# anonymous-author-918/deq-mpc-corl

Hardware: AMD Instinct MI355X
Metric: QP solves/sec at (B,T=20,nx=13,nu=4) (higher is better)
Workload: dtype f32

## Files before the change

### deq-mpc-corl_amd/csrc/alqp_kernels.hip

```cpp
#include <hip/hip_runtime.h>

#include "alqp_team.hpp"
#include "alqp_quad.hpp"
#include "mi_alqp.h"
#include "alqp_dims.hpp"

#ifndef ALQP_PART
#define ALQP_PART 0
#endif
#define ALQP_BUILD_MAIN (ALQP_PART == 0 || ALQP_PART == 1)
#define ALQP_BUILD_QUAD (ALQP_PART == 0 || ALQP_PART == 2 || ALQP_PART == 3)
#define ALQP_QUAD_F32 (ALQP_PART == 0 || ALQP_PART == 2)
#define ALQP_QUAD_F64 (ALQP_PART == 0 || ALQP_PART == 3)

#include <hip/hip_cooperative_groups.h>

namespace alqp {

template <typename real>
struct SolveArgs {
    int B, T;
    int al_iter, max_newton, n_ls, flags;
    real rho_scale;
    const real *Qd, *q, *F, *c, *x0, *ulo, *uhi;
// ... 335 lines not shown
#endif
    QSTAMP(-1);
    if (!(a.flags & ALQP_WS_PRIMED)) {
        if constexpr (NL) qd.stage_in(false, false);
        else qd.stage_in(a.max_newton == 0 || a.al_iter == 0 || (a.flags & ALQP_EXIT_IN_KERNEL) ||
                         (!C::PHI0_FWD && (a.flags & ALQP_INIT_MERIT)));
    }
    const bool ref_exit = (a.flags & ALQP_EXIT_IN_KERNEL) != 0;
    int gphase = 0;

    int step_id = 0;
    bool pend = false;
    real alpha_pend = 0;
    int bad = 0;
    real rn2 = 0, phi_next = 0;
    for (int it = 0; it < a.al_iter; ++it) {
        bool phi_from_forward = false;
        if (a.flags & ALQP_INIT_MERIT) {
            if (it > 0) {
                phi_prev = phi_next;
            } else if (C::PHI0_FWD && a.max_newton > 0 && !ref_exit) {
                phi_from_forward = true;
            } else {
                if constexpr (NL) qd.template linearize<Dyn>(real(0), false);
                real p1[1];
                qd.template merit_candidates<1>(p1, true);
                phi_prev = p1[0];
            }
        }
        pend = false;
        double nrm_old = 0;
        int n_done = 0;
        if (ref_exit) {
            int bad0 = 0;
            const real r0 = it == 0 ? qd.rplus2(bad0) : rn2;
            nrm_old = sqrt(grid_sum_ordered(wave_sum_leaders(exit_term(r0, qor(qd.info)), active && qd.q == 0), a.exit_scratch, gphase));
        }
        for (int st = 0; st < a.max_newton; ++st, ++step_id) {
            real *tg = nullptr;
            if constexpr (TRACE) tg = (tr.g && active) ? tr.g + ((size_t)step_id * a.B + b) * T * N : nullptr;
            QSTAMP(9);
            if constexpr (NL) {
                qd.template linearize<Dyn>(alpha_pend, pend);
                pend = false;
            }
            qd.forward(tg, alpha_pend, pend, (phi_from_forward && st == 0) ? &phi_prev : nullptr);
            real ph[20];
            qd.template backward<FUSE_LS>(ph);
            QSTAMP(-1);
            if constexpr (TRACE) {
                if (tr.d && active) {
                    real *td = tr.d + ((size_t)step_id * a.B + b) * T * N;
                    for (int t = 0; t < T; ++t)
                        for (int j = qd.q; j < N; j += 4) td[t * N + j] = qd.recp(t)[C::oY + C::pn(j)];
                }
            }
            if constexpr (NL) qd.template merit_nonlin<Dyn>(ph);
            else if constexpr (!FUSE_LS) qd.template merit_candidates<20>(ph, false);
            QSTAMP(6);
            int kbest = 0;
            real best = ph[0];
#pragma unroll
            for (int k = 1; k < 20; ++k) {
                if (k < a.n_ls && !(best != best) && (ph[k] != ph[k] || ph[k] < best)) {
                    best = ph[k];
                    kbest = k;
                }
            }
            const bool acc = best < phi_prev;
            if constexpr (TRACE) {
                if (active && qd.q == 0) {
                    if (tr.phi)
#pragma unroll
                        for (int k = 0; k < 20; ++k)
                            if (k < a.n_ls) tr.phi[((size_t)step_id * a.n_ls + k) * a.B + b] = ph[k];
                    if (tr.phi_prev) tr.phi_prev[(size_t)step_id * a.B + b] = phi_prev;
                    if (tr.k) tr.k[(size_t)step_id * a.B + b] = kbest;
                    if (tr.accept) tr.accept[(size_t)step_id * a.B + b] = acc ? 1 : 0;
                }
            }
            const real alpha = acc ? real(1) / real(1 << kbest) : real(0);
            pend = true;
            alpha_pend = alpha;
            QSTAMP(7);
            phi_prev = best;
            if (ref_exit) {
                int bad1 = 0;
                real ph_unused = 0, r1 = 0;
                qd.template iter_end<Dyn>(alpha_pend, pend, false, (real)a.rho_scale, false, ph_unused, r1, bad1);
                pend = false;
                const double nw = sqrt(grid_sum_ordered(wave_sum_leaders(exit_term(r1, qor(qd.info)), active && qd.q == 0), a.exit_scratch, gphase));
                ++n_done;
                if (nw < a.exit_tol || fabs(nrm_old - nw) / nw < a.exit_tol) break;
                nrm_old = nw;
            }
        }
        if (ref_exit && a.newton_counts && blockIdx.x == 0 && lane == 0) a.newton_counts[it] = grid_barrier_timed_out(a.exit_scratch) ? -1 : n_done;
        bad = 0;
        qd.template iter_end<Dyn>(alpha_pend, pend, (a.flags & ALQP_DUAL_UPDATE) != 0, (real)a.rho_scale, it + 1 == a.al_iter,
                    phi_next, rn2, bad);
        pend = false;
    }
    if (a.al_iter <= 0) {
        rn2 = qd.rplus2(bad);
        qd.stage_out();
    }
#ifdef ALQP_PHASE_TIMING
    QSTAMP(9);
    if (lane == 0)
        for (int i = 0; i < 10; ++i) atomicAdd(&g_phase_cycles[i], qd.tacc[i]);
#endif
    if (active && qd.q == 0) {
        a.rho[b] = qd.rho;
        a.phi[b] = phi_prev;
        if (a.rnorm2) a.rnorm2[b] = rn2;
        if (a.info && qd.info && a.info[b] == 0) a.info[b] = qd.info;
        if (a.status) a.status[b] = bad ? 0 : 1;
    }
}

template <typename real, int NX, int NU>
__global__ __launch_bounds__(64) __attribute__((amdgpu_waves_per_eu(1, 1))) void k_backward_quad(BwdArgs<real> a, real *ws) {
    using C = QCfg<real, NX, NU>;
    constexpr int N = C::N;
    const int lane = threadIdx.x, qi = lane >> 2;
    const int b_raw = blockIdx.x * 16 + qi;
    const bool active = b_raw < a.B;
    const int b = active ? b_raw : a.B - 1;
    const int T = a.T;
    Quad<real, NX, NU> qd;
    __shared__ real w_lds[QCfg<real, NX, NU>::WLDS_WORDS];
    qd.wl = w_lds + threadIdx.x;
    qd.q = lane & 3;
    qd.T = T;
    qd.active = active;
    qd.gF = a.F + (size_t)b * (T - 1) * NX * N;
    qd.gQd = nullptr; qd.gq = nullptr; qd.gc = nullptr; qd.gx0 = nullptr; qd.gulo = nullptr; qd.guhi = nullptr;
    qd.st_u = 0;
    qd.gz = nullptr; qd.glam = nullptr;
    qd.rec = ws + C::rec_base(b, T);
    qd.rho = a.rho[b];
    qd.info = 0;
    qd.solve_forward(a.gbar + (size_t)b * T * N);
    real unused[20];
    qd.template backward<false>(unused);
    if (active) {
        const real *zf = a.z_final + (size_t)b * T * N;
        real *qg = a.q_grad + (size_t)b * T * N;
        real *Qg = a.Qd_grad + (size_t)b * T * N;
        for (int t = 0; t < T; ++t)
            for (int j = qd.q; j < N; j += 4) {
                const real w = qd.recp(t)[C::oY + C::pn(j)];
                qg[t * N + j] = w;
                Qg[t * N + j] = w * zf[t * N + j];
            }
    }
}

template <typename real, int NX, int NU>
__global__ __launch_bounds__(64) __attribute__((amdgpu_waves_per_eu(1, 1))) void k_newton_step_quad(StepArgs<real> a, real *ws) {
    using C = QCfg<real, NX, NU>;
    constexpr int N = C::N, SW = C::SW;
    const int lane = threadIdx.x, qi = lane >> 2;
    const int b_raw = blockIdx.x * 16 + qi;
    const bool active = b_raw < a.B;
    const int b = active ? b_raw : a.B - 1;
    const int T = a.T, M = C::M(T) + T * a.nobs;
    Quad<real, NX, NU> qd;
    __shared__ real w_lds[QCfg<real, NX, NU>::WLDS_WORDS];
    qd.wl = w_lds + threadIdx.x;
    qd.q = lane & 3;
    qd.T = T;
    qd.active = active;
    qd.gQd = a.Qd + (size_t)b * T * N;
    qd.gq = a.q + (size_t)b * T * N;
    qd.gF = a.F + (size_t)b * (T - 1) * NX * N;
    qd.gc = nullptr;
    qd.gx0 = a.x0 + (size_t)b * NX;
    qd.gulo = a.ulo + (size_t)b * a.sb_u;
    qd.guhi = a.uhi + (size_t)b * a.sb_u;
    qd.st_u = a.st_u;
    qd.gz = const_cast<real *>(a.z) + (size_t)b * T * N;
    qd.glam = const_cast<real *>(a.lam) + (size_t)b * M;
    qd.rec = ws + C::rec_base(b, T);
    qd.gFw = const_cast<real *>(qd.gF);
    qd.dyn_h = 0;
    qd.rho = a.rho[b];
    qd.info = 0;
    qd.nobs = a.nobs;
    qd.gobs = a.nobs > 0 ? a.obs + (size_t)b * T * a.nobs * 3 : nullptr;
    qd.obs_r2 = a.obs_r2;
    qd.no_init = a.no_init != 0;
    const real *gxn = a.xnext + (size_t)b * (T - 1) * NX;
    real *tg = (a.g_out && active) ? a.g_out + (size_t)b * T * N : nullptr;
    qd.template forward<true>(tg, real(0), false, nullptr, gxn);
    real unused[20];
    qd.template backward<false>(unused, a.d_out + (size_t)b * T * N);
    if (active) {
        if (qd.q == 0 && a.info && qd.info && a.info[b] == 0) a.info[b] = qd.info;
    }
}

#endif

#if ALQP_BUILD_MAIN
// ... 1217 lines not shown
```

### deq-mpc-corl_amd/csrc/alqp_quad.hpp

```cpp
#pragma once
#include <hip/hip_runtime.h>

#include "alqp_team.hpp"
#include "alqp_dyn.hpp"

namespace alqp {

template <int Q>
__device__ inline float qb(float v) {
    return __builtin_bit_cast(float, __builtin_amdgcn_mov_dpp(__builtin_bit_cast(int, v), Q * 0x55, 0xF, 0xF, true));
}
template <int Q>
__device__ inline double qb(double v) {
    long long b = __builtin_bit_cast(long long, v);
    int lo = __builtin_amdgcn_mov_dpp((int)(b & 0xffffffffll), Q * 0x55, 0xF, 0xF, true);
    int hi = __builtin_amdgcn_mov_dpp((int)(b >> 32), Q * 0x55, 0xF, 0xF, true);
    return __builtin_bit_cast(double, ((long long)hi << 32) | (unsigned int)lo);
}
template <typename real>
__device__ inline real qbv(real v, int src) {
    switch (src & 3) {
        case 0: return qb<0>(v);
        case 1: return qb<1>(v);
        case 2: return qb<2>(v);
        default: return qb<3>(v);
    }
}
template <int CTRL>
__device__ inline float qperm(float v) {
    return __builtin_bit_cast(float, __builtin_amdgcn_mov_dpp(__builtin_bit_cast(int, v), CTRL, 0xF, 0xF, true));
}
template <int CTRL>
__device__ inline double qperm(double v) {
    long long b = __builtin_bit_cast(long long, v);
    int lo = __builtin_amdgcn_mov_dpp((int)(b & 0xffffffffll), CTRL, 0xF, 0xF, true);
    int hi = __builtin_amdgcn_mov_dpp((int)(b >> 32), CTRL, 0xF, 0xF, true);
    return __builtin_bit_cast(double, ((long long)hi << 32) | (unsigned int)lo);
}
template <typename real>
__device__ inline real qsum(real v) {
    v += qperm<0xB1>(v);
    v += qperm<0x4E>(v);
    return v;
}
__device__ inline int qor(int v) {
    v |= __builtin_amdgcn_mov_dpp(v, 0xB1, 0xF, 0xF, true);
    v |= __builtin_amdgcn_mov_dpp(v, 0x4E, 0xF, 0xF, true);
    return v;
}
template <typename real>
__device__ inline real sel4(real a0, real a1, real a2, real a3, int q) {
    real lo = (q & 1) ? a1 : a0, hi = (q & 1) ? a3 : a2;
    return (q & 2) ? hi : lo;
}
// ... 14 lines not shown
}
__device__ inline void gst4(double *p, double a, double b, double c, double d) {
    d4u t; t.x = a; t.y = b; t.z = c; t.w = d;
    *reinterpret_cast<d4u *>(p) = t;
}
template <int LEN, typename real>
__device__ inline void gload(const real *p, real (&dst)[LEN]) {
#pragma unroll
    for (int c = 0; c + 4 <= LEN; c += 4) gld4(p + c, dst[c], dst[c + 1], dst[c + 2], dst[c + 3]);
#pragma unroll
    for (int c = (LEN / 4) * 4; c < LEN; ++c) dst[c] = p[c];
}

#ifndef ALQP_W_LDS
#define ALQP_W_LDS 1
#endif
#ifndef ALQP_EXP_NOQ
#define ALQP_EXP_NOQ 0
#endif
#ifndef ALQP_EXP_NORS
#define ALQP_EXP_NORS 0
#endif
#ifndef ALQP_EXP_NOL
#define ALQP_EXP_NOL 0
#endif
template <typename real, int SW, int N, bool IN_LDS>
struct WPanel {
    real a[SW][N];
    __device__ __forceinline__ real (&operator[](int s))[N] { return a[s]; }
    __device__ __forceinline__ const real (&operator[](int s) const)[N] { return a[s]; }
};
template <typename real, int N>
struct WRowLds {
    real *p;
    __device__ __forceinline__ real &operator[](int k) const { return p[k * 64]; }
};
template <typename real, int SW, int N>
struct WPanel<real, SW, N, true> {
    real *base;
    __device__ __forceinline__ WRowLds<real, N> operator[](int s) const { return WRowLds<real, N>{base + s * N * 64}; }
};
template <int LEN, typename real>
__device__ __forceinline__ void gload(const real *p, WRowLds<real, LEN> row) {
    real tmp[LEN];
    gload<LEN>(p, tmp);
#pragma unroll
    for (int k = 0; k < LEN; ++k) row[k] = tmp[k];
}

struct NoDyn {
    static constexpr int ID = 0;
};

template <typename real, int NX_, int NU_>
struct QCfg {
    static constexpr int NX = NX_, NU = NU_, N = NX_ + NU_;
    static constexpr int SH = (N + 3) / 4;
    static constexpr int SW = (NX + 3) / 4;
    static constexpr int SY = SH;
    static constexpr int HT = 2 * SH * (SH + 1);
    __host__ __device__ static constexpr int hidx(int s, int j) { return 2 * s * (s + 1) + j; }
    static constexpr int ST = 2 * SW * (SW + 1);
    static constexpr int NLAST = N - 4 * (SH - 1);
    __host__ __device__ static constexpr int lanes_of(int s) { return s == SH - 1 ? NLAST : 4; }
    __host__ __device__ static constexpr int lbase(int s) {
        int o = 0;
        for (int i = 0; i < s; ++i) o += (i + 1) * 4 * lanes_of(i);
        return o;
    }
    static constexpr int LW = lbase(SH);
    static constexpr bool PHI0_FWD = sizeof(real) == 4;
#ifndef ALQP_S_AFTER_F32
#define ALQP_S_AFTER_F32 0
#endif
    static constexpr bool S_AFTER = sizeof(real) == 8 || ALQP_S_AFTER_F32;
#ifndef ALQP_W_LDS_F32
#define ALQP_W_LDS_F32 0
#endif
    static constexpr bool W_LDS = ALQP_W_LDS && (sizeof(real) == 8 || ALQP_W_LDS_F32);
    static constexpr int WLDS_WORDS = W_LDS ? SW * N * 64 : 1;
    __host__ __device__ static constexpr int p4(int x) { return (x + 3) & ~3; }
    static constexpr int oL = 0;
    static constexpr int oY = oL + p4(LW);
    static constexpr int oR = oY + 4 * SY;
    static constexpr int oS = oR + 4 * SW;
    static constexpr int oZ = oS + 4 * SW;
    static constexpr int oLE = oZ + 4 * SY;
    static_assert(NU <= 4, "the u-slot layout holds one control per lane");
    static constexpr int oUS = oLE + 4 * SW;
    static constexpr int oQ = oUS + 16;
    static constexpr int oq = oQ + 4 * SY;
    static constexpr int oC = oq + 4 * SY;
    static constexpr int RECW = (oC + 4 * SW + 31) & ~31;
    __host__ __device__ static constexpr int pn(int k) { return (k & 3) * SY + (k >> 2); }
    __host__ __device__ static constexpr int px(int r) { return (r & 3) * SW + (r >> 2); }
    __host__ __device__ static constexpr int M(int T) { return T * NX + 2 * T * NU; }
    __host__ __device__ static constexpr size_t rec_base(int b, int T) { return (size_t)b * T * RECW; }
    __host__ __device__ static constexpr size_t ws_words(int B, int T) { return (size_t)B * T * RECW; }
    __host__ static bool ws_covers(int B, int T) { return rec_base(B - 1, T) + (size_t)(T - 1) * RECW + RECW <= ws_words(B, T); }
};

template <typename real, int NX, int NU>
struct Quad {
    using C = QCfg<real, NX, NU>;
    static constexpr int N = C::N, SH = C::SH, SW = C::SW, SY = C::SY, HT = C::HT, ST = C::ST, RECW = C::RECW;

    int q, T;
    bool active;
    const real *gQd, *gq, *gF, *gc, *gx0, *gulo, *guhi;
    long st_u;
    real *gz, *glam, *rec;
    real rho;
    int info;
    real *wl;
    using WT = WPanel<real, SW, N, C::W_LDS>;
    __device__ __forceinline__ WT wpanel() const {
        if constexpr (C::W_LDS) return WT{wl};
        else return WT{};
    }
    real *gFw;
    real dyn_h;
    const real *gobs;
    int nobs;
    real obs_r2;
    bool no_init;

    __device__ __forceinline__ real uhi(int t, int j) const { return guhi[t * st_u + j]; }
    __device__ __forceinline__ real ulo(int t, int j) const { return gulo[t * st_u + j]; }
    __device__ __forceinline__ real *recp(int t) const { return rec + (size_t)t * RECW; }
#ifdef ALQP_PHASE_TIMING
    unsigned long long tacc[10], tlast;
    __device__ __forceinline__ void stamp(int bucket) {
        unsigned long long now;
        __builtin_amdgcn_sched_barrier(0);
        asm volatile("s_waitcnt vmcnt(0)\n\ts_memtime %0\n\ts_waitcnt lgkmcnt(0)" : "=s"(now)::"memory");
        __builtin_amdgcn_sched_barrier(0);
        if (bucket >= 0) tacc[bucket] += now - tlast;
        tlast = now;
    }
#define ALQP_STAMP(b) stamp(b)
#else
#define ALQP_STAMP(b)
#endif

    __device__ __forceinline__ void ld_own_n(const real *field, real (&v)[SY]) const { gload<SY>(field + q * SY, v); }
    __device__ __forceinline__ void ld_own_x(const real *field, real (&v)[SW]) const { gload<SW>(field + q * SW, v); }
    __device__ __forceinline__ void ld_ownx_of_n(const real *field, real (&v)[SW]) const { gload<SW>(field + q * SY, v); }
    template <int LEN>
    __device__ __forceinline__ void gstore(real *p, const real (&v)[LEN]) const {
#pragma unroll
        for (int c = 0; c + 4 <= LEN; c += 4) gst4(p + c, v[c], v[c + 1], v[c + 2], v[c + 3]);
#pragma unroll
        for (int c = (LEN / 4) * 4; c < LEN; ++c) p[c] = v[c];
    }
    __device__ __forceinline__ void st_own_n(real *field, const real (&v)[SY]) const { gstore<SY>(field + q * SY, v); }
    __device__ __forceinline__ void st_own_x(real *field, const real (&v)[SW]) const { gstore<SW>(field + q * SW, v); }
    __device__ __forceinline__ void ld_rep_n(const real *field, real (&v)[N]) const {
        real w[4 * SY];
        gload<4 * SY>(field, w);
#pragma unroll
        for (int k = 0; k < N; ++k) v[k] = w[C::pn(k)];
    }
    __device__ __forceinline__ void ld_repx_of_n(const real *field, real (&v)[NX]) const {
        real w[4 * SY];
        gload<4 * SY>(field, w);
#pragma unroll
        for (int k = 0; k < NX; ++k) v[k] = w[C::pn(k)];
    }
    __device__ __forceinline__ void ld_rep_x(const real *field, real (&v)[NX]) const {
        real w[4 * SW];
        gload<4 * SW>(field, w);
#pragma unroll
        for (int r = 0; r < NX; ++r) v[r] = w[C::px(r)];
    }
    template <int LEN, int SL>
    __device__ __forceinline__ void own_of(const real (&full)[LEN], real (&v)[SL]) const {
#pragma unroll
        for (int m = 0; m < SL; ++m)
            v[m] = (4 * m < LEN) ? sel4(full[(4 * m < LEN) ? 4 * m : 0], (4 * m + 1 < LEN) ? full[(4 * m + 1 < LEN) ? 4 * m + 1 : 0] : real(0),
                                        (4 * m + 2 < LEN) ? full[(4 * m + 2 < LEN) ? 4 * m + 2 : 0] : real(0),
                                        (4 * m + 3 < LEN) ? full[(4 * m + 3 < LEN) ? 4 * m + 3 : 0] : real(0), q)
                                 : real(0);
    }
    template <int LEN, int SL>
    __device__ __forceinline__ void ld_own_ext(const real *src, real (&v)[SL]) const {
#pragma unroll
        for (int m = 0; m < SL; ++m) {
            const int k = 4 * m + q;
            const real x = src[(4 * m + 3 < LEN || k < LEN) ? k : LEN - 1];
            v[m] = (4 * m + 3 < LEN || k < LEN) ? x : real(0);
        }
    }
    template <int LEN, int SL>
    __device__ __forceinline__ void st_own_ext(real *dst, const real (&v)[SL]) const {
#pragma unroll
        for (int m = 0; m < SL; ++m)
            if (4 * m + 3 < LEN || 4 * m + q < LEN) dst[4 * m + q] = v[m];
    }

    __device__ __forceinline__ int own_ju() const { return (q - NX) & 3; }
    __device__ __forceinline__ void ld_own_us(const real *rp, real &lu, real &ll, real &bu, real &bl) const {
        gld4(rp + C::oUS + 4 * q, lu, ll, bu, bl);
    }
    __device__ __forceinline__ void ld_rep_us(const real *rp, real (&lu)[NU], real (&ll)[NU], real (&bu)[NU], real (&bl)[NU]) const {
        real w[16];
        gload<16>(rp + C::oUS, w);
#pragma unroll
        for (int ju = 0; ju < NU; ++ju) {
            const int ql = (NX + ju) & 3;
            lu[ju] = w[4 * ql];
            ll[ju] = w[4 * ql + 1];
            bu[ju] = w[4 * ql + 2];
            bl[ju] = w[4 * ql + 3];
        }
    }

    __device__ __forceinline__ void load_F_rows(int t, WT &W) const {
        const real *Fg = gF + (size_t)t * NX * N;
#pragma unroll
        for (int s = 0; s < SW; ++s) {
            const int r = 4 * s + q;
            const int rc = (4 * s + 3 < NX) ? r : (r < NX ? r : NX - 1);
            gload<N>(Fg + rc * N, W[s]);
            if (4 * s + 3 >= NX) {
                const real m = r < NX ? real(1) : real(0);
#pragma unroll
                for (int k = 0; k < N; ++k) W[s][k] *= m;
            }
        }
    }
    template <int LEN>
    __device__ __forceinline__ void copy_slice(const real *src, real *dst) const {
#pragma unroll
        for (int c = 0; 16 * c < LEN; ++c) {
            const int w0 = 16 * c + 4 * q;
            if (16 * c + 15 < LEN || w0 + 3 < LEN) {
                real a, b, cc, d;
                gld4(src + w0, a, b, cc, d);
                gst4(dst + w0, a, b, cc, d);
            } else {
#pragma unroll
                for (int w = 0; w < 4; ++w)
                    if (w0 + w < LEN) dst[w0 + w] = src[w0 + w];
            }
        }
    }
    __device__ __forceinline__ void stage_in(bool with_residual, bool have_c = true) {
#pragma unroll 2
        for (int t = 0; t < T; ++t) {
            const bool dyn = t < T - 1;
            real *rp = recp(t);
            if (active) {
                real vn[SY], vx[SW];
                ld_own_ext<N>(gz + t * N, vn);
                st_own_n(rp + C::oZ, vn);
                ld_own_ext<N>(gQd + t * N, vn);
                st_own_n(rp + C::oQ, vn);
                ld_own_ext<N>(gq + t * N, vn);
                st_own_n(rp + C::oq, vn);
                ld_own_ext<NX>(glam + t * NX, vx);
                st_own_x(rp + C::oLE, vx);
                {
                    const int ju = own_ju(), jc = ju < NU ? ju : 0;
                    const real *lb = glam + T * NX + t * 2 * NU;
                    const real a0 = lb[jc], a1 = lb[NU + jc], a2 = guhi[t * st_u + jc], a3 = gulo[t * st_u + jc];
                    const bool has = ju < NU;
                    gst4(rp + C::oUS + 4 * q, has ? a0 : real(0), has ? a1 : real(0), has ? a2 : real(0), has ? a3 : real(0));
                }
                if (dyn && have_c) ld_own_ext<NX>(gc + t * NX, vx);
                else {
#pragma unroll
                    for (int s = 0; s < SW; ++s) vx[s] = 0;
                }
                if (have_c) st_own_x(rp + C::oC, vx);
            }
            if (with_residual) {
                WT W = wpanel();
                real zt[N];
                load_F_rows(dyn ? t : (T > 1 ? T - 2 : 0), W);
                gload<N>(gz + t * N, zt);
                real rr[SW];
#pragma unroll
                for (int s = 0; s < SW; ++s) {
                    const int r = 4 * s + q;
                    rr[s] = 0;
                    if (4 * s + 3 < NX || r < NX) {
                        real xn = dyn ? gc[t * NX + r] : real(0);
#pragma unroll
                        for (int k = 0; k < N; ++k) xn = fma_(W[s][k], zt[k], xn);
                        rr[s] = dyn ? gz[(t + 1) * N + r] - xn : gz[r] - gx0[r];
                    }
                }
                if (active) st_own_x(rp + C::oR, rr);
            }
        }
    }
    __device__ __forceinline__ void stage_out() {
        if (!active) return;
#pragma unroll 2
        for (int t = 0; t < T; ++t) {
            const real *rp = recp(t);
            real vn[SY], vx[SW];
            ld_own_n(rp + C::oZ, vn);
            st_own_ext<N>(gz + t * N, vn);
            ld_own_x(rp + C::oLE, vx);
            st_own_ext<NX>(glam + t * NX, vx);
            {
                real lu, ll, bu, bl;
                ld_own_us(rp, lu, ll, bu, bl);
                const int ju = own_ju();
                if (ju < NU) {
                    glam[T * NX + t * 2 * NU + ju] = lu;
                    glam[T * NX + t * 2 * NU + NU + ju] = ll;
                }
            }
        }
    }

    template <class Dyn>
    __device__ __forceinline__ void linearize(real alpha, bool pend) {
// ... 381 lines not shown
                        real wv[KB][SW];
#pragma unroll
                        for (int kk = 0; kk < KB; ++kk)
#pragma unroll
                            for (int s = 0; s < SW; ++s)
                                if (k0 + kk < N) wv[kk][s] = W[s][k0 + kk];
                        __builtin_amdgcn_sched_barrier(0);
#pragma unroll
                        for (int kk = 0; kk < KB; ++kk) {
                            const int k = k0 + kk;
                            if (k < N) {
                                const real lkj = qbv(H[C::hidx(k >> 2, j)], k) * ip;
#pragma unroll
                                for (int s = (k >> 2); s < SH; ++s) H[C::hidx(s, k)] = fma_(-H[C::hidx(s, j)], lkj, H[C::hidx(s, k)]);
#pragma unroll
                                for (int s = 0; s < SW; ++s) W[s][k] = fma_(-wj[s], lkj, wv[kk][s]);
                                Y[k] = fma_(-Y[j], lkj, Y[k]);
                            }
                        }
                    }
                } else {
#pragma unroll
                for (int k = j + 1; k < N; ++k) {
                    const real lkj = qbv(H[C::hidx(k >> 2, j)], k) * ip;
#pragma unroll
                    for (int s = (k >> 2); s < SH; ++s) H[C::hidx(s, k)] = fma_(-H[C::hidx(s, j)], lkj, H[C::hidx(s, k)]);
#pragma unroll
                    for (int s = 0; s < SW; ++s) W[s][k] = fma_(-W[s][j], lkj, W[s][k]);
                    Y[k] = fma_(-Y[j], lkj, Y[k]);
                }
                }
                if constexpr (C::S_AFTER) ipv[j] = ip;
                if (!C::S_AFTER && dyn) {
#pragma unroll
                    for (int b = 0; b < NX; ++b) {
                        const real wbj = qbv(W[b >> 2][j], b) * ip;
#pragma unroll
                        for (int s = (b >> 2); s < SW; ++s) S[C::hidx(s, b)] = fma_(W[s][j], wbj, S[C::hidx(s, b)]);
                    }
                    const real yip = Y[j] * ip;
#pragma unroll
                    for (int s = 0; s < SW; ++s) Sy[s] = fma_(W[s][j], yip, Sy[s]);
                }
                H[C::hidx(j >> 2, j)] = (q == (j & 3)) ? ip : H[C::hidx(j >> 2, j)];
            }
            ALQP_STAMP(2);
            if (active) {
                if (!(ALQP_EXP_NOL && t >= T - ALQP_EXP_NOL))
#pragma unroll
                for (int s = 0; s < SH; ++s)
#pragma unroll
                    for (int c = 0; c <= s; ++c)
                        if (C::lanes_of(s) == 4 || q < C::lanes_of(s))
                            gst4(rp + C::oL + C::lbase(s) + c * 4 * C::lanes_of(s) + 4 * q, H[C::hidx(s, 4 * c)],
                                 H[C::hidx(s, 4 * c + 1)], H[C::hidx(s, 4 * c + 2)], H[C::hidx(s, 4 * c + 3)]);
                real yo[SY];
                own_of<N, SY>(Y, yo);
                st_own_n(rp + C::oY, yo);
                if (pending) st_own_n(rp + C::oZ, zs);
            }

            if constexpr (C::S_AFTER) {
                if (dyn) {
#pragma unroll
                    for (int j = 0; j < N; ++j) {
#pragma unroll
                        for (int b = 0; b < NX; ++b) {
                            const real wbj = qbv(W[b >> 2][j], b) * ipv[j];
#pragma unroll
                            for (int s = (b >> 2); s < SW; ++s) S[C::hidx(s, b)] = fma_(W[s][j], wbj, S[C::hidx(s, b)]);
                        }
                        const real yip = Y[j] * ipv[j];
#pragma unroll
                        for (int s = 0; s < SW; ++s) Sy[s] = fma_(W[s][j], yip, Sy[s]);
                    }
                }
            }
#pragma unroll
            for (int s = 0; s < SW; ++s) {
                vpo[s] = v[s];
                Syo[s] = Sy[s];
            }
            ALQP_STAMP(3);
        }
        if constexpr (C::PHI0_FWD) { if (phi0) *phi0 = qsum(mdist); }
    }

    template <bool LS>
    __device__ __forceinline__ void backward(real (&phi)[20], real *d_ext = nullptr) {
        constexpr int MU0 = NX / 4;
        real c0 = 0, c1 = 0, c2 = 0;
        real acc[20];
        real rvT[SW], lvT[SW];
#pragma unroll
        for (int k = 0; k < 20; ++k) acc[k] = 0;
#pragma unroll
        for (int s = 0; s < SW; ++s) rvT[s] = lvT[s] = 0;
        real dxn[NX];
#pragma unroll
        for (int j = 0; j < NX; ++j) dxn[j] = 0;
        for (int t = T - 1; t >= 0; --t) {
            const bool dyn = t < T - 1;
            real *rp = recp(t);
            real H[HT];
            if (ALQP_EXP_NOL && t >= T - ALQP_EXP_NOL) {
#pragma unroll
                for (int i = 0; i < HT; ++i) H[i] = real(1);
            } else
#pragma unroll
            for (int s = 0; s < SH; ++s)
#pragma unroll
                for (int c = 0; c <= s; ++c) {
                    const int ql = (C::lanes_of(s) == 4 || q < C::lanes_of(s)) ? q : 0;
                    gld4(rp + C::oL + C::lbase(s) + c * 4 * C::lanes_of(s) + 4 * ql, H[C::hidx(s, 4 * c)],
                         H[C::hidx(s, 4 * c + 1)], H[C::hidx(s, 4 * c + 2)], H[C::hidx(s, 4 * c + 3)]);
                }
            real yo[SY];
            ld_own_n(rp + C::oY, yo);
            real Y[N];
#pragma unroll
            for (int j = 0; j < N; ++j) Y[j] = qbv(yo[j >> 2], j);
            WT W = wpanel();
            load_F_rows(dyn ? t : (T > 1 ? T - 2 : 0), W);
            real zz[SY], QQ[SY], qq[SY], rv[SW], lv[SW];
            real lu = 0, ll = 0, bu = 0, bl = 0;
            if constexpr (LS) {
                ld_own_n(rp + C::oZ, zz);
                if constexpr (ALQP_EXP_NOQ) { for (int m = 0; m < SY; ++m) QQ[m] = real(1); }
                else ld_own_n(rp + C::oQ, QQ);
                ld_own_n(rp + C::oq, qq);
                ld_own_us(rp, lu, ll, bu, bl);
                if constexpr (ALQP_EXP_NORS) { for (int s = 0; s < SW; ++s) rv[s] = real(0); }
                else ld_own_x(rp + C::oR, rv);
                ld_own_x(rp + C::oLE, lv);
            }
            ALQP_STAMP(4);
            real dxs[SW];
#pragma unroll
            for (int s = 0; s < SW; ++s)
                dxs[s] = sel4(dxn[4 * s], (4 * s + 1 < NX) ? dxn[(4 * s + 1 < NX) ? 4 * s + 1 : 0] : real(0),
                              (4 * s + 2 < NX) ? dxn[(4 * s + 2 < NX) ? 4 * s + 2 : 0] : real(0),
                              (4 * s + 3 < NX) ? dxn[(4 * s + 3 < NX) ? 4 * s + 3 : 0] : real(0), q);
            if (dyn) {
                real vv[N];
#pragma unroll
                for (int j = 0; j < N; ++j) {
                    real p = 0;
#pragma unroll
                    for (int s = 0; s < SW; ++s) p = fma_(W[s][j], dxs[s], p);
                    vv[j] = qsum(p);
                }
#pragma unroll
                for (int j = 0; j < N; ++j) {
                    const real wj = vv[j] * qbv(H[C::hidx(j >> 2, j)], j);
#pragma unroll
                    for (int k = j + 1; k < N; ++k) vv[k] = fma_(-qbv(H[C::hidx(k >> 2, j)], k), wj, vv[k]);
                }
#pragma unroll
                for (int j = 0; j < N; ++j) Y[j] = fma_(rho, vv[j], Y[j]);
            }
#pragma unroll
            for (int i = N - 1; i >= 0; --i) {
                const real di = Y[i] * qbv(H[C::hidx(i >> 2, i)], i);
                Y[i] = di;
#pragma unroll
                for (int j = 0; j < i; ++j) Y[j] = fma_(-qbv(H[C::hidx(i >> 2, j)], i), di, Y[j]);
            }
// ... 62 lines not shown
#pragma unroll
                    for (int s = 0; s < SW; ++s) {
                        rvT[s] = rv[s];
                        lvT[s] = lv[s];
                    }
                }
            }
#pragma unroll
            for (int j = 0; j < NX; ++j) dxn[j] = Y[j];
            ALQP_STAMP(5);
        }
        if (active && !d_ext) {
            real so[SW];
            own_of<NX, SW>(dxn, so);
            st_own_x(recp(T - 1) + C::oS, so);
        }
        if constexpr (LS) {
#pragma unroll
            for (int s = 0; s < SW; ++s) {
                const int r = 4 * s + q;
                const real ok = (4 * s + 3 < NX || r < NX) ? real(1) : real(0);
                const real sj = sel4(dxn[4 * s], (4 * s + 1 < NX) ? dxn[(4 * s + 1 < NX) ? 4 * s + 1 : 0] : real(0),
                                     (4 * s + 2 < NX) ? dxn[(4 * s + 2 < NX) ? 4 * s + 2 : 0] : real(0),
                                     (4 * s + 3 < NX) ? dxn[(4 * s + 3 < NX) ? 4 * s + 3 : 0] : real(0), q);
                const real rr = rvT[s] * ok, ss = sj * ok, lm = lvT[s] * ok;
                c0 = fma_(fma_(real(0.5) * rho, rr, lm), rr, c0);
                c1 = fma_(fma_(rho, rr, lm), ss, c1);
                c2 = fma_(real(0.5) * rho * ss, ss, c2);
            }
            c0 = qsum(c0);
            c1 = qsum(c1);
            c2 = qsum(c2);
            real alpha = 1;
#pragma unroll
            for (int k = 0; k < 20; ++k) {
                phi[k] = qsum(acc[k]) + fma_(alpha, fma_(alpha, c2, c1), c0);
                alpha *= real(0.5);
            }
        }
    }

    __device__ __forceinline__ void solve_forward(const real *gbar) {
        real e[N];
#pragma unroll
        for (int j = 0; j < N; ++j) e[j] = 0;
        for (int t = 0; t < T; ++t) {
            real *rp = recp(t);
            real H[HT];
#pragma unroll
            for (int s = 0; s < SH; ++s)
#pragma unroll
                for (int c = 0; c <= s; ++c) {
                    const int ql = (C::lanes_of(s) == 4 || q < C::lanes_of(s)) ? q : 0;
                    gld4(rp + C::oL + C::lbase(s) + c * 4 * C::lanes_of(s) + 4 * ql, H[C::hidx(s, 4 * c)],
                         H[C::hidx(s, 4 * c + 1)], H[C::hidx(s, 4 * c + 2)], H[C::hidx(s, 4 * c + 3)]);
                }
            real Y[N];
            gload<N>(gbar + t * N, Y);
            WT W = wpanel();
            load_F_rows(t > 0 ? t - 1 : 0, W);
#pragma unroll
            for (int j = 0; j < N; ++j) Y[j] = -Y[j];
            if (t > 0) {
                real cpl[SW];
#pragma unroll
                for (int s = 0; s < SW; ++s) {
                    real p = 0;
#pragma unroll
                    for (int k = 0; k < N; ++k) p = fma_(W[s][k], e[k], p);
                    cpl[s] = p;
                }
#pragma unroll
                for (int j = 0; j < NX; ++j) Y[j] = fma_(rho, qbv(cpl[j >> 2], j), Y[j]);
            }
#pragma unroll
            for (int j = 0; j < N; ++j) {
                const real yj = Y[j] * qbv(H[C::hidx(j >> 2, j)], j);
#pragma unroll
                for (int k = j + 1; k < N; ++k) Y[k] = fma_(-qbv(H[C::hidx(k >> 2, j)], k), yj, Y[k]);
            }
            if (active) {
                real yo[SY];
                own_of<N, SY>(Y, yo);
                st_own_n(rp + C::oY, yo);
            }
#pragma unroll
            for (int j = 0; j < N; ++j) e[j] = Y[j];
#pragma unroll
            for (int i = N - 1; i >= 0; --i) {
                const real ei = e[i] * qbv(H[C::hidx(i >> 2, i)], i);
                e[i] = ei;
#pragma unroll
                for (int j = 0; j < i; ++j) e[j] = fma_(-qbv(H[C::hidx(i >> 2, j)], i), ei, e[j]);
            }
        }
    }

    template <int K>
    __device__ __forceinline__ void merit_candidates(real (&phi)[K], bool at_z) {
        real c0 = 0, c1 = 0, c2 = 0;
        real acc[K];
#pragma unroll
        for (int k = 0; k < K; ++k) acc[k] = 0;
        constexpr int MU0 = NX / 4;
#pragma unroll 4
        for (int t = 0; t < T; ++t) {
            const real *rp = recp(t);
// ... 86 lines not shown
                if (t < T - 1) {
                    const real *rn_ = recp(t + 1);
                    real zr[N], dr[N], xn[NX];
                    ld_rep_n(rp + C::oZ, zr);
                    ld_rep_n(rp + C::oY, dr);
                    if (pend) {
#pragma unroll
                        for (int k = 0; k < N; ++k) zr[k] = fma_(alpha, dr[k], zr[k]);
                    }
                    dyn_value<Dyn, real>(zr, dyn_h, xn);
                    real zno[SW], dno[SW];
                    ld_ownx_of_n(rn_ + C::oZ, zno);
                    ld_ownx_of_n(rn_ + C::oY, dno);
#pragma unroll
                    for (int s = 0; s < SW; ++s) {
                        real znn = zno[s];
                        const real dnn = dno[s];
                        if (pend) znn = fma_(alpha, dnn, znn);
                        const real xr = sel4(xn[4 * s], (4 * s + 1 < NX) ? xn[(4 * s + 1 < NX) ? 4 * s + 1 : 0] : real(0),
                                             (4 * s + 2 < NX) ? xn[(4 * s + 2 < NX) ? 4 * s + 2 : 0] : real(0),
                                             (4 * s + 3 < NX) ? xn[(4 * s + 3 < NX) ? 4 * s + 3 : 0] : real(0), q);
                        rtrue[s] = znn - xr;
                    }
                }
            }
            real zu = 0;
#pragma unroll
            for (int m = 0; m < SY; ++m) {
                const int j = 4 * m + q;
                const bool valid = 4 * m + 3 < N || j < N;
                const real ok = valid ? real(1) : real(0);
                const real z = valid ? (pend ? fma_(alpha, dd[m], zz[m]) : zz[m]) : real(0);
                const real Qv = QQ[m] * ok, qv = qq[m] * ok;
                if (valid) bad |= !(z - z == real(0));
                zz[m] = z;
                if (valid && active) {
                    if (write_out) gz[t * N + j] = z;
                }
                c0 = fma_(fma_(real(0.5) * Qv, z, qv), z, c0);
                if (m >= MU0) zu = (j >= NX && j < N) ? z : zu;
            }
            {
                const int ju = own_ju();
                const bool isub = ju < NU;
                const real isu = isub ? real(1) : real(0);
                const real vu = zu - bu, vl = bl - zu;
                real lun = lu, lln = ll;
                if (dual) {
                    const real a = fma_(rho, vu, lu), c = fma_(rho, vl, ll);
                    lun = a < 0 ? real(0) : a;
                    lln = c < 0 ? real(0) : c;
                }
                if (isub && active) {
                    if (dual) gst4(rp + C::oUS + 4 * q, lun, lln, bu, bl);
                    if (write_out) {
                        glam[T * NX + t * 2 * NU + ju] = lun;
                        glam[T * NX + t * 2 * NU + NU + ju] = lln;
                    }
                }
                const real cu = fmax_(vu, real(0)), cl = fmax_(vl, real(0));
                acc0 = fma_(isu, fma_(lun, vu, lln * vl) + real(0.5) * rho_n * fma_(cu, cu, cl * cl), acc0);
                r2 = fma_(isu, fma_(cu, cu, cl * cl), r2);
            }
            if (pend && active) st_own_n(rp + C::oZ, zz);
#pragma unroll
            for (int s = 0; s < SW; ++s) {
                const int r = 4 * s + q;
                const bool valid = 4 * s + 3 < NX || r < NX;
                const real ok = valid ? real(1) : real(0);
                real rn = pend ? fma_(alpha, sv[s], rv[s]) : rv[s];
                if constexpr (Dyn::ID != 0) {
                    if (t < T - 1) rn = rtrue[s];
                }
                if (!valid) rn = 0;
                const real ln = valid ? (dual ? fma_(rho, rn, lv[s]) : lv[s]) : real(0);
                rv[s] = rn;
                lv[s] = ln;
                if (valid && active) {
                    if (write_out) glam[t * NX + r] = ln;
                }
                const real rr = rn * ok, lm = ln * ok;
                c0 = fma_(fma_(real(0.5) * rho_n, rr, lm), rr, c0);
                r2 = fma_(rr, rr, r2);
            }
            if (active) {
                if (pend || Dyn::ID != 0) st_own_x(rp + C::oR, rv);
                if (dual) st_own_x(rp + C::oLE, lv);
            }
        }
        rho = rho_n;
        c0 = qsum(c0);
        phi_next = qsum(acc0) + c0;
        rn2 = qsum(r2);
        bad = qor(bad);
    }

    __device__ __forceinline__ real rplus2(int &bad) {
        real acc = 0;
        for (int t = 0; t < T; ++t) {
            const real *rp = recp(t);
            real ro[SW], zo[SY];
            real ulu, ull, ubu, ubl;
            ld_own_x(rp + C::oR, ro);
            ld_own_n(rp + C::oZ, zo);
            ld_own_us(rp, ulu, ull, ubu, ubl);
#pragma unroll
            for (int s = 0; s < SW; ++s) {
// ... 23 lines not shown
```

Measured before the change: 5.317 million.

## Re-lay per-timestep workspace records into lane-interleaved 64-byte groups

Restructures the per-timestep record layout so that each field is stored as 16-word groups in which the four lanes of a quad read contiguous float4 chunks, with leftover slots packed into shared tail groups. For f32 it also interleaves two batch elements' records at 64-byte granularity, so neighbouring quads in a wave touch adjacent cache blocks. Field offsets become typed handles that carry head and tail positions, and all loads and stores go through new slot and field helpers. The aim is more coalesced, cache-line-aligned global traffic in the Riccati forward and backward passes, at the cost of more complex address arithmetic and some padding in the workspace.

```diff
diff --git a/deq-mpc-corl_amd/csrc/alqp_kernels.hip b/deq-mpc-corl_amd/csrc/alqp_kernels.hip
--- a/deq-mpc-corl_amd/csrc/alqp_kernels.hip
+++ b/deq-mpc-corl_amd/csrc/alqp_kernels.hip
@@ -411,7 +411,7 @@
                 if (tr.d && active) {
                     real *td = tr.d + ((size_t)step_id * a.B + b) * T * N;
                     for (int t = 0; t < T; ++t)
-                        for (int j = qd.q; j < N; j += 4) td[t * N + j] = qd.recp(t)[C::oY + C::pn(j)];
+                        for (int j = qd.q; j < N; j += 4) td[t * N + j] = qd.recp(t)[C::wn(C::oY, j)];
                 }
             }
             if constexpr (NL) qd.template merit_nonlin<Dyn>(ph);
@@ -509,7 +509,7 @@
         real *Qg = a.Qd_grad + (size_t)b * T * N;
         for (int t = 0; t < T; ++t)
             for (int j = qd.q; j < N; j += 4) {
-                const real w = qd.recp(t)[C::oY + C::pn(j)];
+                const real w = qd.recp(t)[C::wn(C::oY, j)];
                 qg[t * N + j] = w;
                 Qg[t * N + j] = w * zf[t * N + j];
             }
diff --git a/deq-mpc-corl_amd/csrc/alqp_quad.hpp b/deq-mpc-corl_amd/csrc/alqp_quad.hpp
--- a/deq-mpc-corl_amd/csrc/alqp_quad.hpp
+++ b/deq-mpc-corl_amd/csrc/alqp_quad.hpp
@@ -1,5 +1,7 @@
 #pragma once
 #include <hip/hip_runtime.h>
+
+#include <type_traits>
 
 #include "alqp_team.hpp"
 #include "alqp_dyn.hpp"
@@ -120,6 +122,24 @@
     static constexpr int ID = 0;
 };
 
+struct Fld {
+    int h, t;
+};
+template <int H, int T>
+struct FldT {
+    static constexpr int h = H, t = T;
+    __host__ __device__ constexpr operator Fld() const { return {H, T}; }
+};
+template <typename real>
+struct FRef {
+    real *p;
+    Fld f;
+};
+template <typename real, int H, int T>
+__device__ __forceinline__ FRef<std::remove_const_t<real>> operator+(real *p, FldT<H, T>) {
+    return {const_cast<std::remove_const_t<real> *>(p), Fld{H, T}};
+}
+
 template <typename real, int NX_, int NU_>
 struct QCfg {
     static constexpr int NX = NX_, NU = NU_, N = NX_ + NU_;
@@ -129,11 +149,19 @@
     static constexpr int HT = 2 * SH * (SH + 1);
     __host__ __device__ static constexpr int hidx(int s, int j) { return 2 * s * (s + 1) + j; }
     static constexpr int ST = 2 * SW * (SW + 1);
+    static constexpr int BLK = 64 / (int)sizeof(real);
+#ifndef ALQP_REC_IL_F32
+#define ALQP_REC_IL_F32 2
+#endif
+    static constexpr int IL = sizeof(real) == 4 ? ALQP_REC_IL_F32 : 1;
+    static_assert(IL == 1 || BLK == 16, "groups of 16 words are 64-byte blocks");
+    __host__ __device__ static constexpr int w(int x) { return (x / 16) * (16 * IL) + x % 16; }
     static constexpr int NLAST = N - 4 * (SH - 1);
     __host__ __device__ static constexpr int lanes_of(int s) { return s == SH - 1 ? NLAST : 4; }
+    __host__ __device__ static constexpr int lstride(int s) { return lanes_of(s) == 3 ? 16 : 4 * lanes_of(s); }
     __host__ __device__ static constexpr int lbase(int s) {
         int o = 0;
-        for (int i = 0; i < s; ++i) o += (i + 1) * 4 * lanes_of(i);
+        for (int i = 0; i < s; ++i) o += (i + 1) * lstride(i);
         return o;
     }
     static constexpr int LW = lbase(SH);
@@ -148,24 +176,55 @@
     static constexpr bool W_LDS = ALQP_W_LDS && (sizeof(real) == 8 || ALQP_W_LDS_F32);
     static constexpr int WLDS_WORDS = W_LDS ? SW * N * 64 : 1;
     __host__ __device__ static constexpr int p4(int x) { return (x + 3) & ~3; }
-    static constexpr int oL = 0;
-    static constexpr int oY = oL + p4(LW);
-    static constexpr int oR = oY + 4 * SY;
-    static constexpr int oS = oR + 4 * SW;
-    static constexpr int oZ = oS + 4 * SW;
-    static constexpr int oLE = oZ + 4 * SY;
+    static constexpr int NF = 9;
+    __host__ __device__ static constexpr int fslots(int i) { return (i <= 1 || i == 6 || i == 7) ? SY : (i == 5 ? 4 : SW); }
+    static constexpr int oL = 2 * 16 * (SY / 4);
+    __host__ __device__ static constexpr int tail_at(int i) {
+        int g = (oL + LW + 15) & ~15, o = 0;
+        for (int k = 0; k < NF; ++k) {
+            const int r = fslots(k) % 4;
+            if (r > 0 && o + r > 4) { g += 16; o = 0; }
+            if (k == i) return g + o;
+            o += r;
+        }
+        return o > 0 ? g + 16 : g;
+    }
+    __host__ __device__ static constexpr int head_at(int i) {
+        if (i < 2) return i * 16 * (SY / 4);
+        int o = tail_at(NF);
+        for (int k = 2; k < i; ++k) o += 16 * (fslots(k) / 4);
+        return o;
+    }
+    static constexpr FldT<head_at(0), tail_at(0)> oY{};
+    static constexpr FldT<head_at(1), tail_at(1)> oZ{};
+    static constexpr FldT<head_at(2), tail_at(2)> oR{};
+    static constexpr FldT<head_at(3), tail_at(3)> oS{};
+    static constexpr FldT<head_at(4), tail_at(4)> oLE{};
     static_assert(NU <= 4, "the u-slot layout holds one control per lane");
-    static constexpr int oUS = oLE + 4 * SW;
-    static constexpr int oQ = oUS + 16;
-    static constexpr int oq = oQ + 4 * SY;
-    static constexpr int oC = oq + 4 * SY;
-    static constexpr int RECW = (oC + 4 * SW + 31) & ~31;
-    __host__ __device__ static constexpr int pn(int k) { return (k & 3) * SY + (k >> 2); }
-    __host__ __device__ static constexpr int px(int r) { return (r & 3) * SW + (r >> 2); }
+    static constexpr FldT<head_at(5), tail_at(5)> oUS{};
+    static constexpr FldT<head_at(6), tail_at(6)> oQ{};
+    static constexpr FldT<head_at(7), tail_at(7)> oq{};
+    static constexpr FldT<head_at(8), tail_at(8)> oC{};
+    static constexpr int RECW = (head_at(NF) + 31) & ~31;
+    static_assert(IL == 1 || RECW % 16 == 0, "whole groups per record");
+    template <int S>
+    __host__ __device__ static constexpr int lp(int m, int q) {
+        return m < 4 * (S / 4) ? 16 * (m / 4) + 4 * q + m % 4 : 16 * (S / 4) + q * (S % 4) + m - 4 * (S / 4);
+    }
+    template <int S>
+    __host__ __device__ static constexpr int fw(Fld f, int p) {
+        return p < 16 * (S / 4) ? w(f.h + p) : w(f.t + 4 * ((p - 16 * (S / 4)) / (S % 4)) + (p - 16 * (S / 4)) % (S % 4));
+    }
+    __host__ __device__ static constexpr int pn(int k) { return lp<SY>(k >> 2, k & 3); }
+    __host__ __device__ static constexpr int px(int r) { return lp<SW>(r >> 2, r & 3); }
+    __host__ __device__ static constexpr int wn(Fld f, int k) { return fw<SY>(f, pn(k)); }
     __host__ __device__ static constexpr int M(int T) { return T * NX + 2 * T * NU; }
-    __host__ __device__ static constexpr size_t rec_base(int b, int T) { return (size_t)b * T * RECW; }
-    __host__ __device__ static constexpr size_t ws_words(int B, int T) { return (size_t)B * T * RECW; }
-    __host__ static bool ws_covers(int B, int T) { return rec_base(B - 1, T) + (size_t)(T - 1) * RECW + RECW <= ws_words(B, T); }
+    static constexpr int RSTR = RECW * IL;
+    __host__ __device__ static constexpr size_t rec_base(int b, int T) { return (size_t)(b / IL) * T * RSTR + (size_t)(b % IL) * 16; }
+    __host__ __device__ static constexpr size_t ws_words(int B, int T) { return (size_t)((B + IL - 1) / IL) * T * RSTR; }
+    __host__ static bool ws_covers(int B, int T) {
+        return rec_base(B - 1, T) + (size_t)(T - 1) * RSTR + w(RECW - 1) + 1 <= ws_words(B, T);
+    }
 };
 
 template <typename real, int NX, int NU>
@@ -195,7 +254,7 @@
 
     __device__ __forceinline__ real uhi(int t, int j) const { return guhi[t * st_u + j]; }
     __device__ __forceinline__ real ulo(int t, int j) const { return gulo[t * st_u + j]; }
-    __device__ __forceinline__ real *recp(int t) const { return rec + (size_t)t * RECW; }
+    __device__ __forceinline__ real *recp(int t) const { return rec + (size_t)t * C::RSTR; }
 #ifdef ALQP_PHASE_TIMING
     unsigned long long tacc[10], tlast;
     __device__ __forceinline__ void stamp(int bucket) {
@@ -211,9 +270,46 @@
 #define ALQP_STAMP(b)
 #endif
 
-    __device__ __forceinline__ void ld_own_n(const real *field, real (&v)[SY]) const { gload<SY>(field + q * SY, v); }
-    __device__ __forceinline__ void ld_own_x(const real *field, real (&v)[SW]) const { gload<SW>(field + q * SW, v); }
-    __device__ __forceinline__ void ld_ownx_of_n(const real *field, real (&v)[SW]) const { gload<SW>(field + q * SY, v); }
+    template <int S, int L>
+    __device__ __forceinline__ void ld_slots(FRef<real> f, real (&v)[L]) const {
+        static_assert(L <= S, "slots of the field");
+#pragma unroll
+        for (int c = 0; 4 * c < L && c < S / 4; ++c) {
+            const real *p = f.p + C::w(f.f.h + 16 * c) + 4 * q;
+            if (4 * c + 3 < L) gld4(p, v[4 * c], v[4 * c + 1], v[4 * c + 2], v[4 * c + 3]);
+            else
+#pragma unroll
+                for (int i = 0; 4 * c + i < L; ++i) v[4 * c + i] = p[i];
+        }
+        constexpr int H = 4 * (S / 4), R = S % 4;
+        if constexpr (L > H) {
+            const real *p = f.p + C::w(f.f.t) + 4 * q;
+#pragma unroll
+            for (int m = H; m < L; ++m) v[m] = p[m - H];
+        }
+    }
+    template <int S>
+    __device__ __forceinline__ void st_slots(FRef<real> f, const real (&v)[S]) const {
+#pragma unroll
+        for (int c = 0; c < S / 4; ++c) gst4(f.p + C::w(f.f.h + 16 * c) + 4 * q, v[4 * c], v[4 * c + 1], v[4 * c + 2], v[4 * c + 3]);
+        constexpr int H = 4 * (S / 4), R = S % 4;
+        if constexpr (R > 0) {
+            real *p = f.p + C::w(f.f.t) + 4 * q;
+#pragma unroll
+            for (int m = H; m < S; ++m) p[m - H] = v[m];
+        }
+    }
+    template <int S>
+    __device__ __forceinline__ void ld_field(FRef<real> f, real (&w)[4 * S]) const {
+        constexpr int H = 16 * (S / 4), R = S % 4;
+#pragma unroll
+        for (int c = 0; c < H; c += 4) gld4(f.p + C::w(f.f.h + c), w[c], w[c + 1], w[c + 2], w[c + 3]);
+#pragma unroll
+        for (int i = H; i < H + 4 * R; ++i) w[i] = f.p[C::template fw<S>(f.f, i)];
+    }
+    __device__ __forceinline__ void ld_own_n(FRef<real> f, real (&v)[SY]) const { ld_slots<SY, SY>(f, v); }
+    __device__ __forceinline__ void ld_own_x(FRef<real> f, real (&v)[SW]) const { ld_slots<SW, SW>(f, v); }
+    __device__ __forceinline__ void ld_ownx_of_n(FRef<real> f, real (&v)[SW]) const { ld_slots<SY, SW>(f, v); }
     template <int LEN>
     __device__ __forceinline__ void gstore(real *p, const real (&v)[LEN]) const {
 #pragma unroll
@@ -221,25 +317,28 @@
 #pragma unroll
         for (int c = (LEN / 4) * 4; c < LEN; ++c) p[c] = v[c];
     }
-    __device__ __forceinline__ void st_own_n(real *field, const real (&v)[SY]) const { gstore<SY>(field + q * SY, v); }
-    __device__ __forceinline__ void st_own_x(real *field, const real (&v)[SW]) const { gstore<SW>(field + q * SW, v); }
-    __device__ __forceinline__ void ld_rep_n(const real *field, real (&v)[N]) const {
+    __device__ __forceinline__ void st_own_n(FRef<real> f, const real (&v)[SY]) const { st_slots<SY>(f, v); }
+    __device__ __forceinline__ void st_own_x(FRef<real> f, const real (&v)[SW]) const { st_slots<SW>(f, v); }
+    __device__ __forceinline__ void ld_rep_n(FRef<real> f, real (&v)[N]) const {
         real w[4 * SY];
-        gload<4 * SY>(field, w);
+        ld_field<SY>(f, w);
 #pragma unroll
         for (int k = 0; k < N; ++k) v[k] = w[C::pn(k)];
     }
-    __device__ __forceinline__ void ld_repx_of_n(const real *field, real (&v)[NX]) const {
+    __device__ __forceinline__ void ld_repx_of_n(FRef<real> f, real (&v)[NX]) const {
         real w[4 * SY];
-        gload<4 * SY>(field, w);
+        ld_field<SY>(f, w);
 #pragma unroll
         for (int k = 0; k < NX; ++k) v[k] = w[C::pn(k)];
     }
-    __device__ __forceinline__ void ld_rep_x(const real *field, real (&v)[NX]) const {
+    __device__ __forceinline__ void ld_rep_x(FRef<real> f, real (&v)[NX]) const {
         real w[4 * SW];
-        gload<4 * SW>(field, w);
+        ld_field<SW>(f, w);
 #pragma unroll
         for (int r = 0; r < NX; ++r) v[r] = w[C::px(r)];
+    }
+    __device__ __forceinline__ real *lchunk(real *rp, int s, int c, int ql) const {
+        return rp + C::w(C::oL + C::lbase(s) + c * C::lstride(s)) + 4 * ql;
     }
     template <int LEN, int SL>
     __device__ __forceinline__ void own_of(const real (&full)[LEN], real (&v)[SL]) const {
@@ -268,11 +367,14 @@
 
     __device__ __forceinline__ int own_ju() const { return (q - NX) & 3; }
     __device__ __forceinline__ void ld_own_us(const real *rp, real &lu, real &ll, real &bu, real &bl) const {
-        gld4(rp + C::oUS + 4 * q, lu, ll, bu, bl);
+        gld4(rp + C::w(C::oUS.h) + 4 * q, lu, ll, bu, bl);
+    }
+    __device__ __forceinline__ void st_own_us(real *rp, real lu, real ll, real bu, real bl) const {
+        gst4(rp + C::w(C::oUS.h) + 4 * q, lu, ll, bu, bl);
     }
     __device__ __forceinline__ void ld_rep_us(const real *rp, real (&lu)[NU], real (&ll)[NU], real (&bu)[NU], real (&bl)[NU]) const {
         real w[16];
-        gload<16>(rp + C::oUS, w);
+        ld_field<4>(rp + C::oUS, w);
 #pragma unroll
         for (int ju = 0; ju < NU; ++ju) {
             const int ql = (NX + ju) & 3;
@@ -333,7 +435,7 @@
                     const real *lb = glam + T * NX + t * 2 * NU;
                     const real a0 = lb[jc], a1 = lb[NU + jc], a2 = guhi[t * st_u + jc], a3 = gulo[t * st_u + jc];
                     const bool has = ju < NU;
-                    gst4(rp + C::oUS + 4 * q, has ? a0 : real(0), has ? a1 : real(0), has ? a2 : real(0), has ? a3 : real(0));
+                    st_own_us(rp, has ? a0 : real(0), has ? a1 : real(0), has ? a2 : real(0), has ? a3 : real(0));
                 }
                 if (dyn && have_c) ld_own_ext<NX>(gc + t * NX, vx);
                 else {
@@ -821,7 +923,7 @@
 #pragma unroll
                     for (int c = 0; c <= s; ++c)
                         if (C::lanes_of(s) == 4 || q < C::lanes_of(s))
-                            gst4(rp + C::oL + C::lbase(s) + c * 4 * C::lanes_of(s) + 4 * q, H[C::hidx(s, 4 * c)],
+                            gst4(lchunk(rp, s, c, q), H[C::hidx(s, 4 * c)],
                                  H[C::hidx(s, 4 * c + 1)], H[C::hidx(s, 4 * c + 2)], H[C::hidx(s, 4 * c + 3)]);
                 real yo[SY];
                 own_of<N, SY>(Y, yo);
@@ -881,7 +983,7 @@
 #pragma unroll
                 for (int c = 0; c <= s; ++c) {
                     const int ql = (C::lanes_of(s) == 4 || q < C::lanes_of(s)) ? q : 0;
-                    gld4(rp + C::oL + C::lbase(s) + c * 4 * C::lanes_of(s) + 4 * ql, H[C::hidx(s, 4 * c)],
+                    gld4(lchunk(rp, s, c, ql), H[C::hidx(s, 4 * c)],
                          H[C::hidx(s, 4 * c + 1)], H[C::hidx(s, 4 * c + 2)], H[C::hidx(s, 4 * c + 3)]);
                 }
             real yo[SY];
@@ -1050,7 +1152,7 @@
 #pragma unroll
                 for (int c = 0; c <= s; ++c) {
                     const int ql = (C::lanes_of(s) == 4 || q < C::lanes_of(s)) ? q : 0;
-                    gld4(rp + C::oL + C::lbase(s) + c * 4 * C::lanes_of(s) + 4 * ql, H[C::hidx(s, 4 * c)],
+                    gld4(lchunk(rp, s, c, ql), H[C::hidx(s, 4 * c)],
                          H[C::hidx(s, 4 * c + 1)], H[C::hidx(s, 4 * c + 2)], H[C::hidx(s, 4 * c + 3)]);
                 }
             real Y[N];
@@ -1243,7 +1345,7 @@
                     lln = c < 0 ? real(0) : c;
                 }
                 if (isub && active) {
-                    if (dual) gst4(rp + C::oUS + 4 * q, lun, lln, bu, bl);
+                    if (dual) st_own_us(rp, lun, lln, bu, bl);
                     if (write_out) {
                         glam[T * NX + t * 2 * NU + ju] = lun;
                         glam[T * NX + t * 2 * NU + NU + ju] = lln;
```

New measurement: 5.853 million (median of 6 runs). 10.1% higher.
